# neale/safelife-k2

Hardware: AMD Instinct MI355X
Metric: env-steps/sec (whole node) on 64×64 boards, batch 65536; bit-exact vs CPU ref (higher is better)
Workload: dtype u16; 1 GPU; 64x64 proc-gen prune-still, PPO wrapper chain; envs_per_gpu=65536, burnin_steps=400, global_batch=65536, parallelism=dp1 (env shards), obs=none, rng=philox, board_mode=auto, read_board=False

## Files before the change

### safelife-k2_amd/csrc/sl_bits.hip

```cpp
#include "sl_bits_geo.h"
#include "sl_env_step.h"

using namespace sl;
using namespace sl::fast;
using namespace sl::bits;

namespace {

constexpr int kMinWaves = 4;
constexpr int kMinWavesObs = 3;

constexpr int N = 64;

typedef __attribute__((address_space(3))) u32 lds_u32;

__device__ __forceinline__ void dma_board(const uint16_t *__restrict__ src, lds_u32 *buf,
                                          int lane) {
    const char *s = reinterpret_cast<const char *>(src);
#pragma unroll
    for (int k = 0; k < 8; k++) {
        const int q = k * 64 + lane, row = q >> 3, pos = q & 7;
        const int c = (pos - ((row >> 5) << 2)) & 7;
        __builtin_amdgcn_global_load_lds((const void *)(s + row * 128 + c * 16),
                                         (__attribute__((address_space(3))) void *)(buf + k * 256),
                                         16, 0, 2);
    }
}

__device__ __forceinline__ void read_pairs(const lds_u32 *buf, int lane, u32 D[32]) {
    const int h = lane & 1, j = lane >> 1;
    const lds_u32 *p = buf + h * 1024 + ((j + 16 * h) & 31);
#pragma unroll
    for (int y = 0; y < 32; y++) D[y] = p[y * 32];
}

constexpr int pool_row_plane(int k) { return k < 2 ? 2 * k : 2 * k + 2; }
constexpr bool pool_row_copied(u32 keep, int k) {
    return (((keep & 0xFF85u) >> pool_row_plane(k)) & 3u) != 0u;
}
constexpr int pool_row_slot(u32 keep, bool pack, int k) {
    if (!pack) return k;
    int n = 0;
    for (int i = 0; i < k; i++) n += pool_row_copied(keep, i) ? 1 : 0;
    return n;
}
constexpr int pool_rows_dwords(u32 keep, bool pack) {
    int top = 0;
    for (int k = 0; k < 7; k++)
        if (pool_row_copied(keep, k)) top = pool_row_slot(keep, pack, k) + 1;
    return top * 256;
}
template <u32 KEEP = 0xFFFFu, bool PACK = false>
__device__ __forceinline__ void pool_dma(const sl_level_pool &pool, int li, lds_u32 *buf,
                                         int lane) {
    const char *pl = reinterpret_cast<const char *>(pool.board_planes + (int64_t)li * 16 * N);
    constexpr u32 need = KEEP & 0xFF85u;
#pragma unroll
    for (int k = 0; k < 7; k++) {
        const int p0 = k < 2 ? 2 * k : 2 * k + 2;
        if (!((need >> p0) & 3u)) continue;
        const int slot = PACK ? pool_row_slot(KEEP, true, k) : k;
        __builtin_amdgcn_global_load_lds((const void *)(pl + p0 * N * 8 + lane * 16),
                                         (__attribute__((address_space(3))) void *)(buf + slot * 256),
                                         16, 0, 0);
    }
}
template <u32 KEEP = 0xFFFFu>
__device__ __forceinline__ void pool_planes_lds(const lds_u32 *buf, int dy, int dx, int lane,
                                                u32 S[32]) {
    const int c0 = (2 * (lane >> 1) - dx) & 63, c1 = (c0 + 1) & 63;
    const int r = (32 * (lane & 1) - dy) & 63;
    const bool lo_first = r < 32;
    const u32 sh = (u32)(r & 31);
#pragma unroll
    for (int p = 0; p < 16; p++) {
        if (p == 1 || (p >= 3 && p <= 6) || !((KEEP >> p) & 1u)) {
            PL(S, p, 0) = 0u;
            PL(S, p, 1) = 0u;
            continue;
        }
        const int slot = p < 4 ? p : p - 2;
        const lds_u32 *q = buf + slot * 128;
        const u32 a0 = q[2 * c0], a1 = q[2 * c0 + 1], b0 = q[2 * c1], b1 = q[2 * c1 + 1];
        PL(S, p, 0) = lo_first ? __builtin_amdgcn_alignbit(a1, a0, sh)
                               : __builtin_amdgcn_alignbit(a0, a1, sh);
        PL(S, p, 1) = lo_first ? __builtin_amdgcn_alignbit(b1, b0, sh)
                               : __builtin_amdgcn_alignbit(b0, b1, sh);
    }
}
template <u32 KEEP, int W>
__device__ __forceinline__ void pool_planes_lds_word(const lds_u32 *buf, int dy, int dx,
                                                     int lane, u32 S[32]) {
    const int c = (2 * (lane >> 1) + W - dx) & 63;
    const int r = (32 * (lane & 1) - dy) & 63;
    const bool lo_first = r < 32;
    const u32 sh = (u32)(r & 31);
#pragma unroll
    for (int p = 0; p < 16; p++) {
        if (p == 1 || (p >= 3 && p <= 6) || !((KEEP >> p) & 1u)) {
            PL(S, p, W) = 0u;
            continue;
        }
        const int row = p < 4 ? p >> 1 : (p >> 1) - 1;
        const int slot = 2 * pool_row_slot(KEEP, true, row) + (p & 1);
        const lds_u32 *q = buf + slot * 128;
        const u32 a0 = q[2 * c], a1 = q[2 * c + 1];
        PL(S, p, W) = lo_first ? __builtin_amdgcn_alignbit(a1, a0, sh)
                               : __builtin_amdgcn_alignbit(a0, a1, sh);
    }
}

__device__ __forceinline__ void board_pairs_halves(const uint16_t *__restrict__ src, lds_u32 *buf,
                                                   int lane, u32 D[32]) {
    const int h = lane & 1, j = lane >> 1;
    int l16 = lane * 16;
    asm volatile("" : "+v"(l16));
    const char *s = reinterpret_cast<const char *>(src) + l16;
#pragma unroll
    for (int half = 0; half < 2; half++) {
        wait_lgkm();
        __builtin_amdgcn_fence(__ATOMIC_SEQ_CST, "wavefront");
        __builtin_amdgcn_wave_barrier();
#pragma unroll
        for (int k = 0; k < 4; k++)
            __builtin_amdgcn_global_load_lds((const void *)(s + half * 4096 + k * 1024),
                                             (__attribute__((address_space(3))) void *)(buf + k * 256),
                                             16, 0, 2);
        wait_vm();
        if (h == half) {
#pragma unroll
            for (int y = 0; y < 32; y++) D[y] = buf[y * 32 + j];
        }
    }
    wait_lgkm();
}


typedef __attribute__((address_space(3))) const uint16_t lds_cu16;
struct LdsCells {
    const lds_u32 *buf;
    __device__ __forceinline__ uint32_t operator()(int i) const {
        const int row = i >> 6, col = i & 63;
        const int pos = ((col >> 3) + ((row >> 5) << 2)) & 7;
        return reinterpret_cast<lds_cu16 *>(buf)[row * 64 + pos * 8 + (col & 7)];
    }
};

__device__ __forceinline__ u32 mux_edits(u32 P[32], int ne, const int eidx[4], const u32 eval[4],
                                         int lane) {
    u32 erow = 0;
#pragma unroll
    for (int k = 0; k < 4; k++) {
        if (k < ne) {
            const int y = eidx[k] >> 6, x = eidx[k] & 63;
            const int tl = 2 * (x >> 1) + (y >> 5);
            const u32 bit = 1u << (y & 31);
            const u32 m0 = (lane == tl && !(x & 1)) ? bit : 0u;
            const u32 m1 = (lane == tl && (x & 1)) ? bit : 0u;
            erow |= bit;
#pragma unroll
            for (int p = 0; p < 16; p++) {
                const u32 v = ((eval[k] >> p) & 1u) ? ~0u : 0u;
                PL(P, p, 0) = mux(m0, v, PL(P, p, 0));
                PL(P, p, 1) = mux(m1, v, PL(P, p, 1));
            }
        }
    }
    return erow;
}

__device__ __forceinline__ void wave_reset(const sl_env_state &st, const sl_level_pool &pool,
                                        const ResetArgs &ra, int64_t b, int lane) {
    const int ep = __builtin_amdgcn_readfirstlane(st.episodes[b]);
    const LevelChoice lc = choose_level_wave(pool, ra, ra.env0 + (uint32_t)b, ep, N, N, lane);
    const int li = lc.idx, dy = lc.dy, dx = lc.dx;
    const LevelScalars ls = level_scalars(pool, li);
    const int h = lane & 1, j = lane >> 1;
    const uint16_t *lb = pool.board + (int64_t)li * (N * N), *lg = pool.goals + (int64_t)li * (N * N);
    const int c0 = (2 * j - dx) & 63, c1 = (2 * j + 1 - dx) & 63;
    const int64_t off = b * (int64_t)(N * N);
    const int lane_off = h * 1024 + j;
    u32 *gs = reinterpret_cast<u32 *>(st.start_board + off) + lane_off;
    u32 *gg = reinterpret_cast<u32 *>(st.goals + off) + lane_off;
    u32 *gb = reinterpret_cast<u32 *>(st.board + off) + lane_off;
    auto rolled = [&](const uint16_t *lv, u32 D[32]) {
#pragma unroll
        for (int y = 0; y < 32; y++) {
            const int sr = ((32 * h + y - dy) & 63) * N;
            D[y] = (u32)lv[sr + c0] | ((u32)lv[sr + c1] << 16);
        }
    };
    u32 P[32], D[32];
    rolled(lg, P);
    rolled(lb, D);
#pragma unroll
    for (int y = 0; y < 32; y++) gg[y * 32] = P[y];
    transpose32(P);
    u32 *mg = st.planes ? st.planes + b * 4096 + 2048 + lane : nullptr;
    if (mg) {
#pragma unroll
        for (int q = 0; q < 32; q++) mg[q * 64] = P[q];
    }
    u32 gcol[3][2];
#pragma unroll
    for (int k = 0; k < 3; k++) {
        gcol[k][0] = PL(P, 9 + k, 0);
        gcol[k][1] = PL(P, 9 + k, 1);
    }
    const bool sg = __ballot((PL(P, 7, 0) | PL(P, 7, 1)) != 0u) != 0ull;
#pragma unroll
    for (int y = 0; y < 32; y++) {
        gs[y * 32] = D[y];
        P[y] = D[y];
    }
    transpose32(P);
    int pts, scr, pos, side;
    score_planes(P, gcol, P, &pts, &scr, &pos, &side);
    const ScoreTotals t = score_totals(pts, scr, pos, 0);
    const bool sb = __ballot((PL(P, 7, 0) | PL(P, 7, 1)) != 0u) != 0ull;
    int ev = 0;
    if (lane == 0)
        ev = reset_scalars_from(st, ra, b, li, dy, dx, ls, ep, t.points, t.score, t.possible,
                                (sb ? 1 : 0) | (sg ? 2 : 0));
    ev = __builtin_amdgcn_readfirstlane(ev);
    const u32 ex0 = PL(P, 8, 0), ex1 = PL(P, 8, 1);
    {
#pragma unroll
        for (int y = 0; y < 32; y++) {
            u32 d = D[y];
            if (d & (u32)EXIT) d = (d & 0xFFFF0000u) | (u32)ev;
            if (d & ((u32)EXIT << 16)) d = (d & 0x0000FFFFu) | ((u32)ev << 16);
            gb[y * 32] = d;
        }
    }
    const int n_exit = wave_total(__builtin_popcount(ex0) + __builtin_popcount(ex1));
    {
        u32 e0 = ex0, e1 = ex1;
        const int kmax = n_exit < SL_MAX_EXITS ? n_exit : SL_MAX_EXITS;
        for (int k = 0; k < kmax; k++) {
            const u32 k0 = e0 ? (u32)((32 * h + __builtin_ctz(e0)) * N + 2 * j) : 0xFFFFu;
            const u32 k1 = e1 ? (u32)((32 * h + __builtin_ctz(e1)) * N + 2 * j + 1) : 0xFFFFu;
            u32 m = k0 < k1 ? k0 : k1;
            m = min(m, dpp<0xB1>(m));
            m = min(m, dpp<0x4E>(m));
            m = min(m, dpp<0x141>(m));
            m = min(m, dpp<0x140>(m));
            const u32 key = min(min((u32)__builtin_amdgcn_readlane((int)m, 0),
                                    (u32)__builtin_amdgcn_readlane((int)m, 16)),
                                min((u32)__builtin_amdgcn_readlane((int)m, 32),
                                    (u32)__builtin_amdgcn_readlane((int)m, 48)));
            if (k0 == key) e0 &= e0 - 1;
            if (k1 == key) e1 &= e1 - 1;
            if (lane == 0) {
                st.exit_y[b * SL_MAX_EXITS + k] = (int16_t)(key >> 6);
                st.exit_x[b * SL_MAX_EXITS + k] = (int16_t)(key & 63);
            }
        }
    }
    if (lane == 0) {
        if (mg) st.planes_ok[b] = SL_POK_GOALS_MIRROR;
        st.exit_count[b] = n_exit;
        for (int e = n_exit; e < SL_MAX_EXITS; e++) {
            st.exit_y[b * SL_MAX_EXITS + e] = 0;
            st.exit_x[b * SL_MAX_EXITS + e] = 0;
        }
    }
}

struct StepKArgs {
    sl_env_state st;
    StepArgs a;
    FastExtra fx;
    const int32_t *actions;
    int ctp, ctc;
    double *reward_out;
    uint8_t *done_out, *flags_out;
    int32_t *ep_len_out, *ep_rew_out;
};

__device__ __forceinline__ const StepKArgs &kernarg() {
    auto kp = __builtin_amdgcn_kernarg_segment_ptr();
    asm volatile("" : "+s"(kp));
    return *(const StepKArgs *)kp;
}

__device__ __forceinline__ void lds_put_board(lds_u32 *buf, int lane, const u32 D[32]) {
    const int h = lane & 1, j = lane >> 1;
    lds_u32 *p = buf + h * 1024 + ((j + 16 * h) & 31);
#pragma unroll
    for (int y = 0; y < 32; y++) p[y * 32] = D[y];
}

__device__ __forceinline__ int lds_cell_idx(int row, int col) {
    return row * 64 + ((col + 32 * (row >> 5)) & 63);
}

typedef __attribute__((address_space(3))) uint16_t lds_u16;

__device__ __forceinline__ uint64_t changed_rows64(u32 cl) {
    u32 x = cl | dpp<0x4E>(cl);
    x |= dpp<0x124>(x);
    x |= dpp<0x128>(x);
    const u32 lo = (u32)__builtin_amdgcn_readlane((int)x, 0) | (u32)__builtin_amdgcn_readlane((int)x, 16) |
                   (u32)__builtin_amdgcn_readlane((int)x, 32) | (u32)__builtin_amdgcn_readlane((int)x, 48);
    const u32 hi = (u32)__builtin_amdgcn_readlane((int)x, 1) | (u32)__builtin_amdgcn_readlane((int)x, 17) |
                   (u32)__builtin_amdgcn_readlane((int)x, 33) | (u32)__builtin_amdgcn_readlane((int)x, 49);
    return ((uint64_t)hi << 32) | lo;
}

typedef uint32_t u32x4 __attribute__((ext_vector_type(4)));
__device__ __forceinline__ void store_rows(lds_u32 *buf, uint8_t *rowlist, u32 *gb0, uint64_t M,
                                           u32 keep, int lane) {
    typedef __attribute__((address_space(3))) uint8_t lds_u8;
    typedef __attribute__((address_space(3))) u32x4 lds_u32x4;
    lds_u8 *rl = (lds_u8 *)rowlist;
    if ((M >> lane) & 1ull) rl[lanes_below(M)] = (uint8_t)lane;
    __builtin_amdgcn_fence(__ATOMIC_SEQ_CST, "wavefront");
    __builtin_amdgcn_wave_barrier();
    const int n = __builtin_popcountll(M);
    const int c = lane & 7;
    for (int s = lane >> 3; s < n; s += 8) {
// ... 319 lines not shown
    if (VIEW && hi && !(fx.fuse_reset && reset)) {
        wait_vm();
        const FastExtra &lfx = kernarg().fx;
        sl::obs::ObsArgs oa{};
        oa.vh = lfx.obs_vh;
        oa.vw = lfx.obs_vw;
        oa.remove_white = lfx.obs_rw;
        oa.mode = lfx.obs_mode;
        oa.nch = lfx.obs_nch;
        if (CH)
            sl::obs::obs_channels_wave<obs_esz(OBS)>(
                st, oa, sl::obs::ChanMap{lfx.obs_chpack, lfx.obs_nch}, lfx.obs_one, b, lane, vm,
                reinterpret_cast<uint8_t *>(lfx.obs_out));
        else
            sl::obs::obs_packed_wave(st, oa, b, lane, lfx.obs_out);
    }
    if (fx.fuse_reset && reset && lane == 0) queue_reset(fx.scratch, st.B, a.step, b);
}

template <int OBS, int MODE>
__global__ void __launch_bounds__(64, (OBS || MODE == SPAWN_STREAM) ? kMinWavesObs : kMinWaves)
k_env_step_bits64(StepKArgs ka) {
    const int64_t b = blockIdx.x;
    const int lane = threadIdx.x;
    __shared__ __attribute__((aligned(16))) u32 stage[N * N / 2];
    __shared__ __attribute__((aligned(16))) uint16_t vmask[OBS >= 2 ? sl::obs::kFusedChanCells : 2];
    __shared__ uint8_t rowlist[OBS ? 64 : 1];
    lds_u32 *buf = (lds_u32 *)&stage[0];
    Pre pre;
    issue_pre(ka.st, ka.actions, b, lane, pre);
    dma_board(ka.st.board + b * (int64_t)(N * N), buf, lane);
    step_env<OBS, MODE>(ka.st, ka.a, ka.fx, b, lane, buf, vmask, rowlist, ka.actions, ka.ctp, ka.ctc,
                        ka.reward_out, ka.done_out, ka.flags_out, ka.ep_len_out, ka.ep_rew_out,
                        pre);
}


constexpr u32 kKeepAll = 0xFFFFu, kKeepC3 = 0x877Fu, kAgentC3 = 0x0062u;
constexpr u32 kDerivable = 0x8100u;
__host__ __device__ constexpr u32 derived_eff(u32 derived) {
    return (derived & kDerivable) == kDerivable ? kDerivable : 0u;
}
template <u32 K16, int DM = -1>
struct PlaneSlots {
    static constexpr bool kFixed = K16 == kKeepC3;
    u32 keep;
    u32 store;
    u32 drv_;
    __device__ __forceinline__ u32 drv16() const { return DM >= 0 ? (u32)DM : drv_; }
    __device__ __forceinline__ u32 keep32() const { return K16 ? K16 * 0x10001u : keep; }
    __device__ __forceinline__ u32 store32() const {
        return kFixed ? (K16 & ~kAgentC3) * 0x10001u : store;
    }
    static constexpr bool late(int q) { return (kDerivable >> (q & 15)) & 1u; }
    __device__ __forceinline__ bool kept(int q) const { return (keep32() >> q) & 1u; }
    __device__ __forceinline__ bool laid(int q) const { return (store32() >> q) & 1u; }
    __device__ __forceinline__ bool stored(int q) const {
        return laid(q) && !(late(q) && ((drv16() >> (q & 15)) & 1u));
    }
    __device__ __forceinline__ u32 stored32() const { return store32() & ~(drv16() * 0x10001u); }
    __device__ __forceinline__ u32 agent16() const {
        return kFixed ? kAgentC3 : (keep32() & ~store32()) & 0xFFFFu;
    }
    __device__ __forceinline__ int pos(int q) const {
        const u32 below = (1u << q) - 1u;
        if (kFixed && DM >= 0) return __builtin_popcount(stored32() & below);
        u32 k = stored32();
        asm volatile("" : "+s"(k));
        return __builtin_popcount(k & below);
    }
    __device__ __forceinline__ int stored16() const {
        return __builtin_popcount(stored32() & 0xFFFFu);
    }
    static __device__ __forceinline__ PlaneSlots of(u32 zero, u32 agent, u32 derived) {
        const u32 k = ~zero & 0xFFFFu;
        const u32 s = kFixed ? (K16 & ~kAgentC3) : ((K16 ? K16 : k) & ~agent);
        return PlaneSlots{k * 0x10001u, (k & ~agent) * 0x10001u, derived_eff(derived) & s};
    }
};
__device__ __forceinline__ void exit_words(u32 V, int lane, u32 ew[2]) {
    const RecFields fl{V, 0, 0, 0, 0.0};
    const int n = min(fl.exit_count(), SL_MAX_EXITS);
    ew[0] = ew[1] = 0u;
#pragma unroll 1
    for (int e = 0; e < n; e++) {
        const int y = fl.exit_y(e), x = fl.exit_x(e);
        const u32 bit = lane == 2 * (x >> 1) + (y >> 5) ? 1u << (y & 31) : 0u;
        if (x & 1) ew[1] |= bit;
        else ew[0] |= bit;
    }
}
__device__ __forceinline__ void agent_words(int ay, int ax, int lane, u32 aw[2]) {
    const u32 bit = lane == 2 * (ax >> 1) + (ay >> 5) ? 1u << (ay & 31) : 0u;
    aw[0] = (ax & 1) ? 0u : bit;
    aw[1] = (ax & 1) ? bit : 0u;
}
constexpr int kMinWavesPlanes = 5;
constexpr int planes_min_waves(u32 k16, int obs) {
    return (obs == 0 && k16 == kKeepC3) ? kMinWavesPlanes : kMinWaves;
}

template <u32 K16, int DM>
__device__ __forceinline__ void dma_planes(const u32 *__restrict__ bp, PlaneSlots<K16, DM> ps,
                                           lds_u32 *buf, int lane) {
    const int groups = (2 * ps.stored16() + 3) >> 2;
    const char *s = reinterpret_cast<const char *>(bp);
#pragma unroll
    for (int g = 0; g < 8; g++)
        if (g < groups)
            __builtin_amdgcn_global_load_lds((const void *)(s + g * 1024 + lane * 16),
                                             (__attribute__((address_space(3))) void *)(buf + g * 256),
                                             16, 0, 2);
}

__device__ __forceinline__ int near_cell_index(int k, int y0, int x0) {
    const int dy = k < 5 ? 0 : (k == 5 ? -1 : k == 6 ? 1 : k == 7 ? -2 : 2);
    const int dx = k >= 5 || k == 0 ? 0 : (k == 1 ? -1 : k == 2 ? 1 : k == 3 ? -2 : 2);
    return ((y0 + dy) & 63) * 64 + ((x0 + dx) & 63);
}
struct NearCells {
    int y0, x0;
    u32 v;
    __device__ __forceinline__ uint32_t operator()(int i) const {
        const int dy = (((i >> 6) - y0 + 32) & 63) - 32, dx = (((i & 63) - x0 + 32) & 63) - 32;
        const int k = dy == 0 ? (dx == 0 ? 0 : dx == -1 ? 1 : dx == 1 ? 2 : dx == -2 ? 3 : 4)
                              : (dy == -1 ? 5 : dy == 1 ? 6 : dy == -2 ? 7 : 8);
        return (u32)__builtin_amdgcn_readlane((int)v, __builtin_amdgcn_readfirstlane(k));
    }
};
template <u32 K16, int DM>
__device__ __forceinline__ u32 lds_plane_cell(const lds_u32 *buf, PlaneSlots<K16, DM> ps, u32 V,
                                              int i) {
    const int y = i >> 6, x = i & 63;
    const lds_u32 *q = buf + 2 * (x >> 1) + (y >> 5);
    const u32 r = (u32)(y & 31);
    const int w = 16 * (x & 1);
    u32 v = 0;
#pragma unroll
    for (int p = 0; p < 16; p++) {
        const int pw = ps.pos(p) + (w ? ps.stored16() : 0);
        if (ps.stored(p)) v |= ((q[pw * 64] >> r) & 1u) << p;
    }
    if (ps.drv16() & 0x8000u) v |= (v & 4u) << 13;
    if (ps.drv16() & 0x0100u) {
        const RecFields fl{V, 0, 0, 0, 0.0};
        const int n = min(fl.exit_count(), SL_MAX_EXITS);
#pragma unroll 1
        for (int e = 0; e < n; e++)
            if (i == fl.exit_y(e) * 64 + fl.exit_x(e)) v |= 0x0100u;
    }
    return v;
}

constexpr int planes_dm(u32 k16) { return k16 == kKeepC3 ? (int)kDerivable : -1; }
template <u32 K16, int OBS>
__global__ void __launch_bounds__(64, planes_min_waves(K16, OBS))
k_env_step_bits64_planes(StepKArgs ka) {
    __shared__ __attribute__((aligned(16))) u32 stage[N * N / 2];
    uint16_t *const vm = nullptr;
    constexpr bool GRAY = false, W6 = false, SPLIT_EPI = false;
    constexpr int DM = planes_dm(K16);
#include "sl_planes64_step.inc"
}

template <u32 K16, int OBS>
__global__ void __launch_bounds__(64, planes_min_waves(K16, OBS))
k_env_planes64_gray(StepKArgs ka) {
    static_assert(OBS <= 1, "channel views load the three colour planes");
    __shared__ __attribute__((aligned(16))) u32 stage[N * N / 2];
    uint16_t *const vm = nullptr;
    constexpr bool GRAY = true, W6 = false, SPLIT_EPI = false;
    constexpr int DM = planes_dm(K16);
#include "sl_planes64_step.inc"
}

constexpr int kMinWavesW6 = 6;
constexpr int kStageDwW6 = 1536;
template <u32 K16>
__global__ void __launch_bounds__(64, kMinWavesW6)
k_env_planes64_w6(StepKArgs ka) {
    __shared__ __attribute__((aligned(16))) u32 stage[kStageDwW6];
    uint16_t *const vm = nullptr;
    constexpr int OBS = 0;
    constexpr bool GRAY = true, W6 = true, SPLIT_EPI = false;
    constexpr int DM = planes_dm(K16);
#include "sl_planes64_step.inc"
}

template <u32 K16>
__global__ void __launch_bounds__(64, kMinWavesW6)
k_env_planes64_s6(StepKArgs ka) {
    __shared__ __attribute__((aligned(16))) u32 stage[kStageDwW6];
    uint16_t *const vm = nullptr;
    constexpr int OBS = 0;
    constexpr bool GRAY = true, W6 = true, SPLIT_EPI = true;
    constexpr int DM = planes_dm(K16);
#include "sl_planes64_step.inc"
}

constexpr int kTailThreads = 256;
__global__ void __launch_bounds__(kTailThreads)
k_env_epilogue_reset64(sl_env_state st, StepArgs a, sl_level_pool pool, ResetArgs ra,
                       int64_t *scratch, double *reward_out, uint8_t *done_out,
                       uint8_t *flags_out, int32_t *ep_len_out, int32_t *ep_rew_out) {
    const int64_t b = (int64_t)blockIdx.x * kTailThreads + threadIdx.x;
    const int lane = threadIdx.x & 63;
    if (b == 0) scratch[8 * st.B + 2 + ((a.step + 1) & 1)] = 0;
    bool reset = false;
    if (b < st.B) {
        const Handover h = get_handover(handover_of(scratch, st.B), b);
        const HandFields f{{st, b, a.bonus_table}, h.go, h.ax, h.ay};
        reset = epilogue_core(st, a, b, f, h.act_reward, h.points, h.score, h.possible, h.side,
                              reward_out, done_out, flags_out, ep_len_out, ep_rew_out);
    }
    __shared__ uint64_t finished[kTailThreads / 64];
    const int wave = __builtin_amdgcn_readfirstlane((int)(threadIdx.x >> 6));
    const uint64_t mine = __ballot(reset);
    if (lane == 0) finished[wave] = mine;
    __builtin_amdgcn_fence(__ATOMIC_RELEASE, "workgroup");
    __syncthreads();
    const int64_t b0 = (int64_t)blockIdx.x * kTailThreads;
    int i = 0;
#pragma unroll 1
    for (int q = 0; q < kTailThreads / 64; q++) {
        const uint64_t f = finished[q];
        uint64_t todo = ((uint64_t)(u32)__builtin_amdgcn_readfirstlane((int)(f >> 32)) << 32) |
                        (u32)__builtin_amdgcn_readfirstlane((int)f);
        while (todo) {
            const int k = __builtin_ctzll(todo);
            todo &= todo - 1;
            if ((i++ & (kTailThreads / 64 - 1)) == wave) wave_reset(st, pool, ra, b0 + 64 * q + k, lane);
        }
    }
}

template <u32 K16, int ESZ>
__global__ void __launch_bounds__(64, kMinWaves)
k_env_planes64_chan(StepKArgs ka) {
    constexpr int OBS = ESZ == 1 ? 3 : (ESZ == 4 ? 4 : 2);
    __shared__ __attribute__((aligned(16))) u32 stage[N * N / 2];
    __shared__ __attribute__((aligned(16))) uint16_t vmask[sl::obs::kFusedChanCells];
    uint16_t *const vm = vmask;
    constexpr bool GRAY = false, W6 = false, SPLIT_EPI = false;
    constexpr int DM = planes_dm(K16);
#include "sl_planes64_step.inc"
}

constexpr int stored16_min_waves(int kind, int obs) {
    return kind == 2 || kind == 3 ? kMinWavesW6 : (kind == 4 ? kMinWaves : planes_min_waves(kKeepC3, obs));
}
template <int KIND, int OBS>
__global__ void __launch_bounds__(64, stored16_min_waves(KIND, OBS))
k_env_p64_stored16(StepKArgs ka) {
    constexpr u32 K16 = kKeepC3;
    constexpr int DM = 0;
    constexpr bool GRAY = KIND >= 1 && KIND <= 3, W6 = KIND == 2 || KIND == 3, SPLIT_EPI = KIND == 3;
    __shared__ __attribute__((aligned(16))) u32 stage[W6 ? kStageDwW6 : N * N / 2];
    __shared__ __attribute__((aligned(16))) uint16_t vmask[OBS >= 2 ? sl::obs::kFusedChanCells : 2];
    uint16_t *const vm = OBS >= 2 ? vmask : nullptr;
#include "sl_planes64_step.inc"
}

__global__ void __launch_bounds__(64) k_board_sync64(sl_env_state st, int demote) {
    const int64_t b = blockIdx.x;
    const int lane = threadIdx.x;
    const int pok = __builtin_amdgcn_readfirstlane(st.planes_ok[b]);
    if (!(pok & SL_POK_BOARD_PLANES)) return;
    if (!(pok & SL_POK_BOARD_FULL)) {
        const PlaneSlots<0> ps = PlaneSlots<0>::of(st.board_zero, st.agent_planes,
                                                   st.derived_planes);
        const u32 *bp = st.planes + b * 4096 + lane;
        u32 P[32];
#pragma unroll
        for (int q = 0; q < 32; q++) P[q] = ps.stored(q) ? bp[ps.pos(q) * 64] : 0u;
        u32 aw[2];
        agent_words(__builtin_amdgcn_readfirstlane(st.agent_y[b]),
                    __builtin_amdgcn_readfirstlane(st.agent_x[b]), lane, aw);
#pragma unroll
        for (int q = 0; q < 32; q++)
            if ((ps.agent16() >> (q & 15)) & 1u) P[q] = aw[q >> 4];
        if (ps.drv16() & 0x8000u) {
            PL(P, 15, 0) = PL(P, 2, 0);
            PL(P, 15, 1) = PL(P, 2, 1);
        }
        if (ps.drv16() & 0x0100u) {
            const int n = min(__builtin_amdgcn_readfirstlane(st.exit_count[b]), SL_MAX_EXITS);
            PL(P, 8, 0) = PL(P, 8, 1) = 0u;
            for (int e = 0; e < n; e++) {
                const int y = __builtin_amdgcn_readfirstlane(st.exit_y[b * SL_MAX_EXITS + e]);
                const int x = __builtin_amdgcn_readfirstlane(st.exit_x[b * SL_MAX_EXITS + e]);
                const u32 bit = lane == 2 * (x >> 1) + (y >> 5) ? 1u << (y & 31) : 0u;
                if (x & 1) PL(P, 8, 1) |= bit;
                else PL(P, 8, 0) |= bit;
            }
        }
        transpose32(P);
        u32 *gb = reinterpret_cast<u32 *>(st.board + b * (int64_t)(N * N)) + (lane & 1) * 1024 +
                  (lane >> 1);
#pragma unroll
        for (int y = 0; y < 32; y++) gb[y * 32] = P[y];
    }
    if (lane == 0)
        st.planes_ok[b] = demote ? pok & ~(SL_POK_BOARD_PLANES | SL_POK_BOARD_FULL)
                                 : pok | SL_POK_BOARD_FULL;
}

// ... 226 lines not shown
```

### safelife-k2_amd/csrc/sl_planes64_step.inc

```
    const sl_env_state &st = ka.st;
    const StepArgs &a = ka.a;
    const FastExtra &fx = ka.fx;
    const int64_t b = blockIdx.x;
    const int lane = threadIdx.x;
    lds_u32 *buf = (lds_u32 *)&stage[0];
    const PlaneSlots<K16, DM> ps = PlaneSlots<K16, DM>::of(st.board_zero, st.agent_planes,
                                                           st.derived_planes);
    constexpr int kStageDw = (int)(sizeof(stage) / sizeof(u32));
    static_assert(!W6 || (PlaneSlots<K16, DM>::kFixed && OBS == 0), "W6: fixed planes, no views");
    constexpr int kStoredWords =
        2 * __builtin_popcount(K16 & ~kAgentC3 & ~(u32)(DM > 0 ? DM : 0) & 0xFFFFu);
    static_assert(K16 != kKeepC3 || kStoredWords == (DM ? 12 : 16), "three DMA groups, or four");
    static_assert(!W6 || kStoredWords * 64 <= kStageDw, "the stored plane words fit the buffer");
    static_assert(pool_rows_dwords(K16 ? K16 : 0xFFFFu, W6) <= kStageDw,
                  "the pool's start-plane rows fit the buffer");
    static_assert(kStageDw >= (W6 ? N * N / 4 : N * N / 2), "a board, or half of one (W6)");
    Pre pre;
    const bool gray_blank = GRAY && (!OBS || fx.obs_rw != 0);
    if (!GRAY) issue_pre(st, ka.actions, b, lane, pre);
    else if (gray_blank) issue_pre<0>(st, ka.actions, b, lane, pre);
    else issue_pre<1>(st, ka.actions, b, lane, pre);
    dma_planes(st.planes + b * 4096, ps, buf, lane);
    const int64_t off = b * (int64_t)(N * N);
    const int lane_off = (lane & 1) * 1024 + (lane >> 1);
    u32 *gg = reinterpret_cast<u32 *>(st.goals + off) + lane_off;
    u32 *mg = st.planes + b * 4096 + 2048 + lane;
    u32 *bp = st.planes + b * 4096 + lane;
    const u32 V = pre.V;
    const int pok_all = rec(V, R_POK);
    const bool pin = (pok_all & SL_POK_BOARD_PLANES) != 0;
    u32 gcol[3][2];
#pragma unroll
    for (int k = 0; k < 3; k++) {
        gcol[k][0] = pre.g[k][0];
        gcol[k][1] = pre.g[k][1];
    }
    const int pok = pok_all & kPokGoalsSkip;

    const SpawnCtx sc = spawn_ctx(a, b, rec(V, R_SPAWN));
    const StreamSrc ssrc{a.draws, a.n_draws, nullptr, a.draw_mask, a.draw_bits};

    int gok = pok;
    if ((pok & kPokGoalsSkip) != kPokGoalsSkip)
        gok = goals_step64<true, SPAWN_PHILOX>(gg, mg, pok, lane, sc, ssrc, 0, gcol);
    __builtin_amdgcn_sched_barrier(0);

    int roll = -1;
    if (fx.pool.K > 0 && fx.pool.board_planes && st.start_roll) roll = rec(V, R_ROLL);
    wait_vm();
    if (!pin) {
        if (!W6) {
            dma_board(st.board + off, buf, lane);
            wait_vm();
        }
        u32 R[32];
        if (W6) board_pairs_halves(st.board + off, buf, lane, R);
        else read_pairs(buf, lane, R);
        transpose32(R);
#pragma unroll
        for (int q = 0; q < 32; q++)
            if (ps.stored(q)) buf[ps.pos(q) * 64 + lane] = R[q];
        __builtin_amdgcn_fence(__ATOMIC_SEQ_CST, "wavefront");
        __builtin_amdgcn_wave_barrier();
    }
    RecEnv env{st, b, rec(V, R_GO), rec(V, R_AX), rec(V, R_AY), rec(V, R_SCORE),
               rec(V, R_BASE), rec(V, R_POSS), rec_f64(V, R_MP)};
    int act_reward = 0;
    int eidx[4];
    u32 eval[4];
    const int ay0 = rec(V, R_AY), ax0 = rec(V, R_AX);
    const u32 near = lane < 9 ? lds_plane_cell(buf, ps, V, near_cell_index(lane, ay0, ax0)) |
                                    (lane == 0 ? ps.agent16() : 0u)
                              : 0u;
    OverlayT<NearCells> ov;
    ov.src = NearCells{ay0, ax0, near};
    ov.n = 0;
#pragma unroll
    for (int k = 0; k < 4; k++) {
        ov.idx[k] = 0;
        ov.val[k] = 0;
    }
    if (lane == 0) act_reward = act_core(env, rec(V, R_ACT), N, N, ka.ctp, ka.ctc, ov);
    int ne = ov.n;
#pragma unroll
    for (int k = 0; k < 4; k++) {
        eidx[k] = ov.idx[k];
        eval[k] = ov.val[k];
    }
    act_reward = __builtin_amdgcn_readfirstlane(act_reward);
    ne = __builtin_amdgcn_readfirstlane(ne);
#pragma unroll
    for (int k = 0; k < 4; k++) {
        eidx[k] = __builtin_amdgcn_readfirstlane(eidx[k]);
        eval[k] = (u32)__builtin_amdgcn_readfirstlane((int)eval[k]);
        if (K16) eval[k] &= K16;
        eval[k] &= ~ps.agent16();
    }
    const RecFields fl = rec_fields(a, V, __builtin_amdgcn_readfirstlane(env.go),
                                    __builtin_amdgcn_readfirstlane(env.ax),
                                    __builtin_amdgcn_readfirstlane(env.ay));

    u32 PB[32];
#pragma unroll
    for (int q = 0; q < 32; q++) PB[q] = ps.stored(q) ? buf[ps.pos(q) * 64 + lane] : 0u;
    wait_lgkm();
    constexpr u32 KEEP = K16 ? K16 : 0xFFFFu;
    if (roll < 0) {
        if (!W6) dma_board(st.start_board + off, buf, lane);
    } else pool_dma<KEEP, W6>(fx.pool, rec(V, R_LI), buf, lane);
    (void)mux_edits(PB, ne, eidx, eval, lane);
    {
        u32 aw[2];
        agent_words(fl.ay, fl.ax, lane, aw);
#pragma unroll
        for (int q = 0; q < 32; q++)
            if ((ps.agent16() >> (q & 15)) & 1u) PB[q] = aw[q >> 4];
    }
    if (ps.drv16() & 0x8000u) {
#pragma unroll
        for (int w = 0; w < 2; w++) PL(PB, 15, w) = PL(PB, 2, w);
    }
    if (ps.drv16() & 0x0100u) {
        u32 ew[2];
        exit_words(V, lane, ew);
#pragma unroll
        for (int w = 0; w < 2; w++) PL(PB, 8, w) = ew[w];
    }
    u32 cb[2], held[2];
    rule_planes(PB, cb, Geo64<SPAWN_PHILOX>{lane, ssrc, 0, 0}, sc, 0u, held);
    const uint64_t held_lanes = __ballot((held[0] | held[1]) != 0u);
#pragma unroll
    for (int w = 0; w < 2; w++) asm volatile("" : "+v"(PL(PB, 3, w)));
    __builtin_amdgcn_sched_barrier(0);

    u32 PS[32];
    wait_vm();
    if (roll >= 0) {
        if (!W6) pool_planes_lds<KEEP>(buf, roll >> 16, roll & 0xFFFF, lane, PS);
    } else {
        if (W6) board_pairs_halves(st.start_board + off, buf, lane, PS);
        else read_pairs(buf, lane, PS);
        transpose32(PS);
#pragma unroll
        for (int q = 0; q < 32; q++)
            if (!((KEEP >> (q & 15)) & 1u)) PS[q] = 0u;
    }
    int pts, scr, pos, side;
    const u32 gblack[3][2] = {{0u, 0u}, {0u, 0u}, {0u, 0u}};
    if (W6 && roll >= 0) {
        const int dy = roll >> 16, dx = roll & 0xFFFF;
        int p1, s1, o1, e1;
        pool_planes_lds_word<KEEP, 0>(buf, dy, dx, lane, PS);
        score_planes<false, 0, 1>(PB, GRAY ? gblack : gcol, PS, &pts, &scr, &pos, &side);
        __builtin_amdgcn_sched_barrier(0);
        pool_planes_lds_word<KEEP, 1>(buf, dy, dx, lane, PS);
        score_planes<false, 1, 2>(PB, GRAY ? gblack : gcol, PS, &p1, &s1, &o1, &e1);
        pts += p1;
        scr += s1;
        pos += o1;
        side += e1;
    } else
    score_planes(PB, GRAY ? gblack : gcol, PS, &pts, &scr, &pos, &side);
    const ScoreTotals tot = score_totals(pts, scr, pos, side);
    __builtin_amdgcn_sched_barrier(0);

    const Words2 d9 = recolour_exits(
        PB, can_exit_now(fl.min_performance(), tot.score, fl.baseline(), tot.possible));
    u32 em[2] = {0u, 0u};
#pragma unroll
    for (int k = 0; k < 4; k++) {
        if (k < ne) {
            const int y = eidx[k] >> 6, x = eidx[k] & 63;
            const u32 bit = lane == 2 * (x >> 1) + (y >> 5) ? 1u << (y & 31) : 0u;
            em[x & 1] |= bit;
        }
    }
    u32 dw[2], dall[2];
#pragma unroll
    for (int w = 0; w < 2; w++) {
        dw[w] = cb[w] | em[w];
        dall[w] = em[w] | (((held_lanes >> lane) & 1ull) ? cb[w] : 0u);
    }
    if (!pin || wave_or(dw[0] | dw[1] | d9.w[0] | d9.w[1])) {
#pragma unroll
        for (int k = 0; k < 16; k++) {
            if (!ps.stored(k)) continue;
#pragma unroll
            for (int w = 0; w < 2; w++) {
                const u32 d = (k == 0 || k == 3 || k == 10 || k == 11) ? dw[w]
                              : k == 9 ? (dw[w] | d9.w[w]) : dall[w];
                if (!pin || d)
                    __builtin_nontemporal_store(PL(PB, k, w), &bp[ps.pos(k + 16 * w) * 64]);
            }
        }
    }
    const int ok = gok | SL_POK_BOARD_PLANES;
    if (ok != pok_all && lane == 0) st.planes_ok[b] = ok;
    if (OBS) {
        const bool rw = kernarg().fx.obs_rw != 0;
#pragma unroll
        for (int w = 0; w < 2; w++) {
            if (GRAY && rw) continue;
            u32 g0 = gcol[0][w], g1 = gcol[GRAY ? 0 : 1][w], g2 = gcol[GRAY ? 0 : 2][w];
            if (rw) {
                const u32 wh = g0 & g1 & g2;
                g0 &= ~wh;
                g1 &= ~wh;
                g2 &= ~wh;
            }
            const u32 b12 = PL(PB, 12, w), b13 = PL(PB, 13, w), b14 = PL(PB, 14, w);
            u32 c = b12 & g0;
            PL(PB, 12, w) = b12 ^ g0;
            const u32 x13 = b13 ^ g1;
            PL(PB, 13, w) = x13 ^ c;
            c = (b13 & g1) | (c & x13);
            const u32 x14 = b14 ^ g2;
            PL(PB, 14, w) = x14 ^ c;
            c = (b14 & g2) | (c & x14);
            PL(PB, 15, w) ^= c;
        }
        transpose32(PB);
        lds_put_board(buf, lane, PB);
        __builtin_amdgcn_fence(__ATOMIC_SEQ_CST, "wavefront");
        __builtin_amdgcn_wave_barrier();
        __builtin_amdgcn_sched_barrier(0);
        if (OBS >= 2) write_obs_channels<obs_esz(OBS)>(buf, vm, fl, b, lane);
        else write_obs(buf, fx, fl, b, lane);
        __builtin_amdgcn_sched_barrier(0);
    }
    if (SPLIT_EPI) {
        if (lane == 0)
            put_handover(handover_of(fx.scratch, st.B), b,
                         Handover{act_reward, tot.points, tot.score, tot.possible, tot.side,
                                  fl.go, fl.ax, fl.ay});
    } else {
    int reset = 0;
    if (lane == 0)
        reset = epilogue_core(st, a, b, fl, act_reward, tot.points, tot.score, tot.possible,
                              tot.side, ka.reward_out, ka.done_out, ka.flags_out, ka.ep_len_out,
                              ka.ep_rew_out);
    reset = __builtin_amdgcn_readfirstlane(reset);
    if (fx.fuse_reset && reset && lane == 0) queue_reset(fx.scratch, st.B, a.step, b);
    }
```

Before: 656.2 million env-steps/s.

## Replace single-lane action logic with branch-free four-cell wave-uniform action resolver

For kernels with a fixed plane set, the agent action is now computed branch-free from the four cells along the facing direction. Those cells are read in parallel by four lanes, and exit membership is tested across lanes with a ballot. This replaces the serial lane-0 act_core call over a 9-cell neighbourhood overlay and the chain of readfirstlane broadcasts. The edit mask becomes a per-cell changed bitmask. The cost is new logic that must stay bit-exact with the reference action semantics, including pulls, pushes, toggles and exits.

```diff
diff --git a/safelife-k2_amd/csrc/sl_action4.h b/safelife-k2_amd/csrc/sl_action4.h
--- /dev/null
+++ b/safelife-k2_amd/csrc/sl_action4.h
@@ -0,0 +1,63 @@
+#pragma once
+#include <stdint.h>
+
+#if defined(__HIPCC__)
+#define SL_ACT4_FN __host__ __device__ inline __attribute__((always_inline))
+#else
+#define SL_ACT4_FN inline
+#endif
+
+namespace sl {
+namespace act4 {
+
+constexpr uint32_t kAlive = 0x0001, kPushable = 0x0004, kDestr = 0x0008, kPreserve = 0x0020;
+constexpr uint32_t kInhibit = 0x0040, kSpawn = 0x0080, kExit = 0x0100, kColors = 0x0E00;
+constexpr uint32_t kPullable = 0x8000;
+constexpr uint32_t kLife = kAlive | kDestr;
+constexpr uint32_t kPowers = kAlive | kInhibit | kPreserve | kSpawn;
+
+struct Result {
+    int reward;
+    int game_over;
+    int moved;
+    int orient;
+    int store_orient;
+    int store_agent;
+    uint32_t n[4];
+    uint32_t changed;
+};
+
+SL_ACT4_FN Result action4(int a, int game_over, bool can_exit, int ctp, int ctc, uint32_t c0,
+                          uint32_t c1, uint32_t c2, uint32_t c3) {
+    const bool active = !game_over && a >= 1 && a <= 8;
+    const bool mv = active && a <= 4, tg = active && a > 4;
+    const bool empty = c1 == 0;
+    const bool enter = !empty && (c1 & kExit) && can_exit;
+    const bool push = !empty && !enter && (c1 & kPushable);
+    const bool push_empty = push && c3 == 0;
+    const bool push_exit = push && c3 != 0 && (c3 & kExit);
+    const bool moved = mv && (empty || push_empty || push_exit);
+    const bool pull = moved && (c2 & kPullable);
+    const bool create = tg && c1 == 0;
+    const bool destroy = tg && c1 != 0 && (c1 & kDestr);
+    const bool txor = tg && !create && !destroy;
+    const uint32_t tbits = (ctp ? kPowers : 0u) | (ctc ? kColors : 0u);
+
+    Result r;
+    r.reward = (mv && enter) ? 1 : 0;
+    r.game_over = r.reward ? 1 : game_over;
+    r.moved = moved ? 1 : 0;
+    r.orient = (a - 1) & 3;
+    r.store_orient = active ? 1 : 0;
+    r.store_agent = mv ? 1 : 0;
+    r.n[0] = moved ? (pull ? c2 : 0u) : (txor ? c0 ^ (c1 & tbits) : c0);
+    r.n[1] = moved ? c0 : (create ? (kLife | (c0 & kColors)) : (destroy ? 0u : c1));
+    r.n[2] = pull ? 0u : c2;
+    r.n[3] = (mv && push_empty) ? c1 : c3;
+    r.changed = (r.n[0] != c0 ? 1u : 0u) | (r.n[1] != c1 ? 2u : 0u) | (r.n[2] != c2 ? 4u : 0u) |
+                (r.n[3] != c3 ? 8u : 0u);
+    return r;
+}
+
+}
+}
diff --git a/safelife-k2_amd/csrc/sl_bits.hip b/safelife-k2_amd/csrc/sl_bits.hip
--- a/safelife-k2_amd/csrc/sl_bits.hip
+++ b/safelife-k2_amd/csrc/sl_bits.hip
@@ -1,5 +1,6 @@
 #include "sl_bits_geo.h"
 #include "sl_env_step.h"
+#include "sl_action4.h"
 
 using namespace sl;
 using namespace sl::fast;
@@ -167,6 +168,25 @@
         }
     }
     return erow;
+}
+__device__ __forceinline__ void mux_edits4(u32 P[32], u32 changed, const int eidx[4],
+                                           const u32 eval[4], int lane) {
+#pragma unroll
+    for (int k = 0; k < 4; k++) {
+        if ((changed >> k) & 1u) {
+            const int y = eidx[k] >> 6, x = eidx[k] & 63;
+            const int tl = 2 * (x >> 1) + (y >> 5);
+            const u32 bit = 1u << (y & 31);
+            const u32 m0 = (lane == tl && !(x & 1)) ? bit : 0u;
+            const u32 m1 = (lane == tl && (x & 1)) ? bit : 0u;
+#pragma unroll
+            for (int p = 0; p < 16; p++) {
+                const u32 v = ((eval[k] >> p) & 1u) ? ~0u : 0u;
+                PL(P, p, 0) = mux(m0, v, PL(P, p, 0));
+                PL(P, p, 1) = mux(m1, v, PL(P, p, 1));
+            }
+        }
+    }
 }
 
 __device__ __forceinline__ void wave_reset(const sl_env_state &st, const sl_level_pool &pool,
@@ -792,6 +812,23 @@
     return v;
 }
 
+template <u32 K16, int DM>
+__device__ __forceinline__ u32 lds_plane_cell_stored(const lds_u32 *buf, PlaneSlots<K16, DM> ps,
+                                                     int i) {
+    const int y = i >> 6, x = i & 63;
+    const lds_u32 *q = buf + 2 * (x >> 1) + (y >> 5);
+    const u32 r = (u32)(y & 31);
+    const int w = 16 * (x & 1);
+    u32 v = 0;
+#pragma unroll
+    for (int p = 0; p < 16; p++) {
+        const int pw = ps.pos(p) + (w ? ps.stored16() : 0);
+        if (ps.stored(p)) v |= ((q[pw * 64] >> r) & 1u) << p;
+    }
+    if (ps.drv16() & 0x8000u) v |= (v & 4u) << 13;
+    return v;
+}
+
 constexpr int planes_dm(u32 k16) { return k16 == kKeepC3 ? (int)kDerivable : -1; }
 template <u32 K16, int OBS>
 __global__ void __launch_bounds__(64, planes_min_waves(K16, OBS))
diff --git a/safelife-k2_amd/csrc/sl_planes64_step.inc b/safelife-k2_amd/csrc/sl_planes64_step.inc
--- a/safelife-k2_amd/csrc/sl_planes64_step.inc
+++ b/safelife-k2_amd/csrc/sl_planes64_step.inc
@@ -47,6 +47,38 @@
 
     int roll = -1;
     if (fx.pool.K > 0 && fx.pool.board_planes && st.start_roll) roll = rec(V, R_ROLL);
+    constexpr bool ACT4 = K16 != 0;
+    static_assert(N >= 5 && (N & (N - 1)) == 0, "the four cells are distinct; wrapped by mask");
+    const int act = rec(V, R_ACT), go0 = rec(V, R_GO);
+    const int ay0 = rec(V, R_AY), ax0 = rec(V, R_AX);
+    int eidx[4] = {0, 0, 0, 0};
+    int cell_i = 0;
+    u32 exit_hits = 0u;
+    bool can_exit0 = false;
+    if (ACT4) {
+        const int orient = (act - 1) & 3;
+        const int fdx = orient == 1 ? 1 : (orient == 3 ? -1 : 0);
+        const int fdy = orient == 0 ? -1 : (orient == 2 ? 1 : 0);
+#pragma unroll
+        for (int k = 0; k < 4; k++) {
+            const int d = k == 2 ? -1 : (k == 3 ? 2 : k);
+            eidx[k] = ((ay0 + d * fdy) & (N - 1)) * N + ((ax0 + d * fdx) & (N - 1));
+        }
+        cell_i = (lane & 2) ? ((lane & 1) ? eidx[3] : eidx[2])
+                            : ((lane & 1) ? eidx[1] : eidx[0]);
+        if (ps.drv16() & 0x0100u) {
+            const int e = (lane >> 2) & 7;
+            const int sh = 16 * (e & 1);
+            const int ey = (int)(int16_t)(
+                __builtin_amdgcn_ds_bpermute(4 * (R_EY + (e >> 1)), (int)V) >> sh);
+            const int ex = (int)(int16_t)(
+                __builtin_amdgcn_ds_bpermute(4 * (R_EX + (e >> 1)), (int)V) >> sh);
+            const int n = min(rec(V, R_EXC), SL_MAX_EXITS);
+            exit_hits = (u32)__ballot(lane < 32 && e < n && ey * N + ex == cell_i);
+        }
+        can_exit0 = can_exit_now(rec_f64(V, R_MP), rec(V, R_SCORE), rec(V, R_BASE),
+                                 rec(V, R_POSS));
+    }
     wait_vm();
     if (!pin) {
         if (!W6) {
@@ -63,42 +95,69 @@
         __builtin_amdgcn_fence(__ATOMIC_SEQ_CST, "wavefront");
         __builtin_amdgcn_wave_barrier();
     }
-    RecEnv env{st, b, rec(V, R_GO), rec(V, R_AX), rec(V, R_AY), rec(V, R_SCORE),
-               rec(V, R_BASE), rec(V, R_POSS), rec_f64(V, R_MP)};
-    int act_reward = 0;
-    int eidx[4];
+    int act_reward = 0, go1 = go0, ax1 = ax0, ay1 = ay0;
+    u32 echg = 0u;
     u32 eval[4];
-    const int ay0 = rec(V, R_AY), ax0 = rec(V, R_AX);
-    const u32 near = lane < 9 ? lds_plane_cell(buf, ps, V, near_cell_index(lane, ay0, ax0)) |
-                                    (lane == 0 ? ps.agent16() : 0u)
-                              : 0u;
-    OverlayT<NearCells> ov;
-    ov.src = NearCells{ay0, ax0, near};
-    ov.n = 0;
+    if (ACT4) {
+        const u32 cell_v = lds_plane_cell_stored(buf, ps, cell_i);
+        u32 cell[4];
+#pragma unroll
+        for (int k = 0; k < 4; k++) {
+            cell[k] = (u32)__builtin_amdgcn_readlane((int)cell_v, k);
+            if ((ps.drv16() & 0x0100u) && (exit_hits & (0x11111111u << k))) cell[k] |= EXIT;
+        }
+        cell[0] |= ps.agent16();
+        const act4::Result ar = act4::action4(act, go0, can_exit0, ka.ctp, ka.ctc, cell[0],
+                                              cell[1], cell[2], cell[3]);
+        act_reward = ar.reward;
+        go1 = ar.game_over;
+        if (ar.moved) {
+            ax1 = eidx[1] & (N - 1);
+            ay1 = eidx[1] / N;
+        }
+        if (lane == 0) {
+            if (ar.store_orient) st.orientation[b] = ar.orient;
+            if (ar.reward) st.game_over[b] = 1;
+            if (ar.store_agent) {
+                st.agent_x[b] = ax1;
+                st.agent_y[b] = ay1;
+            }
+        }
+        echg = ar.changed;
+#pragma unroll
+        for (int k = 0; k < 4; k++) eval[k] = ar.n[k];
+    } else {
+        RecEnv env{st, b, go0, ax0, ay0, rec(V, R_SCORE), rec(V, R_BASE), rec(V, R_POSS),
+                   rec_f64(V, R_MP)};
+        const u32 near = lane < 9 ? lds_plane_cell(buf, ps, V, near_cell_index(lane, ay0, ax0)) |
+                                        (lane == 0 ? ps.agent16() : 0u)
+                                  : 0u;
+        OverlayT<NearCells> ov;
+        ov.src = NearCells{ay0, ax0, near};
+        ov.n = 0;
+#pragma unroll
+        for (int k = 0; k < 4; k++) {
+            ov.idx[k] = 0;
+            ov.val[k] = 0;
+        }
+        if (lane == 0) act_reward = act_core(env, act, N, N, ka.ctp, ka.ctc, ov);
+        act_reward = __builtin_amdgcn_readfirstlane(act_reward);
+        echg = (1u << __builtin_amdgcn_readfirstlane(ov.n)) - 1u;
+#pragma unroll
+        for (int k = 0; k < 4; k++) {
+            eidx[k] = __builtin_amdgcn_readfirstlane(ov.idx[k]);
+            eval[k] = (u32)__builtin_amdgcn_readfirstlane((int)ov.val[k]);
+        }
+        go1 = __builtin_amdgcn_readfirstlane(env.go);
+        ax1 = __builtin_amdgcn_readfirstlane(env.ax);
+        ay1 = __builtin_amdgcn_readfirstlane(env.ay);
+    }
 #pragma unroll
     for (int k = 0; k < 4; k++) {
-        ov.idx[k] = 0;
-        ov.val[k] = 0;
-    }
-    if (lane == 0) act_reward = act_core(env, rec(V, R_ACT), N, N, ka.ctp, ka.ctc, ov);
-    int ne = ov.n;
-#pragma unroll
-    for (int k = 0; k < 4; k++) {
-        eidx[k] = ov.idx[k];
-        eval[k] = ov.val[k];
-    }
-    act_reward = __builtin_amdgcn_readfirstlane(act_reward);
-    ne = __builtin_amdgcn_readfirstlane(ne);
-#pragma unroll
-    for (int k = 0; k < 4; k++) {
-        eidx[k] = __builtin_amdgcn_readfirstlane(eidx[k]);
-        eval[k] = (u32)__builtin_amdgcn_readfirstlane((int)eval[k]);
         if (K16) eval[k] &= K16;
         eval[k] &= ~ps.agent16();
     }
-    const RecFields fl = rec_fields(a, V, __builtin_amdgcn_readfirstlane(env.go),
-                                    __builtin_amdgcn_readfirstlane(env.ax),
-                                    __builtin_amdgcn_readfirstlane(env.ay));
+    const RecFields fl = rec_fields(a, V, go1, ax1, ay1);
 
     u32 PB[32];
 #pragma unroll
@@ -108,7 +167,7 @@
     if (roll < 0) {
         if (!W6) dma_board(st.start_board + off, buf, lane);
     } else pool_dma<KEEP, W6>(fx.pool, rec(V, R_LI), buf, lane);
-    (void)mux_edits(PB, ne, eidx, eval, lane);
+    mux_edits4(PB, echg, eidx, eval, lane);
     {
         u32 aw[2];
         agent_words(fl.ay, fl.ax, lane, aw);
@@ -169,7 +228,7 @@
     u32 em[2] = {0u, 0u};
 #pragma unroll
     for (int k = 0; k < 4; k++) {
-        if (k < ne) {
+        if ((echg >> k) & 1u) {
             const int y = eidx[k] >> 6, x = eidx[k] & 63;
             const u32 bit = lane == 2 * (x >> 1) + (y >> 5) ? 1u << (y & 31) : 0u;
             em[x & 1] |= bit;
```

After: 670.0 million env-steps/s, median of 6. 2.1% higher.
